# E3SM-Project/tinman_sandbox

Measured on NVIDIA B200. Metric: compute_and_apply_rhs_elem_lev_updates_per_s, higher is better.
Workload: dtype f64

## Files before the change

tinman_sandbox_b200/csrc/caar_capi.cu:

```cuda
#include <cstdarg>
#include <cstddef>
#include <cstdio>
#include <cstdlib>
#include <cstring>
#include <initializer_list>
#include <new>

#include "caar_device.cuh"

#ifndef CAAR_HOST_DEFAULT_ZERO_COPY
#define CAAR_HOST_DEFAULT_ZERO_COPY 0
#endif

namespace {

thread_local char g_err[512] = "";

int fail(int code, const char* fmt, ...) {
  va_list ap;
  va_start(ap, fmt);
  vsnprintf(g_err, sizeof g_err, fmt, ap);
  va_end(ap);
  return code;
}
// ... 37 lines not shown
  unsigned long long* bits;
  double* out3;
  double* out3_host;
  cudaEvent_t ev0, ev1;
  long long launches;
  caar::TmaMaps* tma;
  cudaStream_t s_in, s_in2, s_out;
  cudaEvent_t* chunk_ev;
  int n_chunk_ev;
  cudaEvent_t ev_fence;
  int rsplit;
  double* hybi_dev;
  double* extra[5];
  double* stage;
  unsigned* lapflat_sched;
  caar::TmaMaps* tma_host;
  double* tma_host_key[CAAR_NUM_FIELDS];
};

static_assert(sizeof(caar_arrays) == CAAR_NUM_FIELDS * sizeof(double*), "caar_arrays must be 16 pointers");
static_assert(sizeof(caar_dims) == 20 && offsetof(caar_dims, nlev) == 4 && offsetof(caar_dims, ntl) == 16, "caar_dims: 5 ints");
static_assert(offsetof(caar_arrays, elem_state_dp3d) == 48 && offsetof(caar_arrays, elem_derived_vn0) == 120,
              "caar_arrays: the order of struct Arrays");
static_assert(sizeof(caar_constants) == 48 && offsetof(caar_constants, kappa) == 40, "caar_constants: 6 doubles");
static_assert(sizeof(caar_control) == 32 && offsetof(caar_control, qn0) == 20 && offsetof(caar_control, dt2) == 24,
              "caar_control: 6 ints + 1 double");
static_assert(sizeof(caar_checksum) == 184 && offsetof(caar_checksum, sumsq) == 56 && offsetof(caar_checksum, bits) == 112 &&
                  offsetof(caar_checksum, energy) == 168,
              "caar_checksum: 7 + 7 doubles, 7 64-bit integers, 2 doubles");

// ... 46 lines not shown
  a.metdet = ptr[4]; a.rmetdet = ptr[5]; a.dp3d = ptr[6]; a.v = ptr[7];
  a.T = ptr[8]; a.phis = ptr[9]; a.Qdp = ptr[10]; a.eta_dot_dpdn = ptr[11];
  a.omega_p = ptr[12]; a.phi = ptr[13]; a.pecnd = ptr[14]; a.vn0 = ptr[15];
  a.nelem = h->dims.nelem; a.nlev = h->dims.nlev; a.qsize_d = h->dims.qsize_d; a.ntl = h->dims.ntl;
  if (ctl) {
    a.nets = ctl->nets; a.nete = ctl->nete; a.n0 = ctl->n0; a.np1 = ctl->np1; a.nm1 = ctl->nm1;
    a.qn0 = ctl->qn0; a.dt2 = ctl->dt2;
  }
  a.rrearth = h->c.rrearth; a.eta_ave_w = h->c.eta_ave_w; a.Rwv = h->c.Rwater_vapor; a.Rgas = h->c.Rgas;
  a.kappa = h->c.kappa; a.hyai0 = h->hyai0; a.ps0 = h->ps0;
  for (int i = 0; i < 16; ++i) a.dvv[i] = h->dvv[i];
  a.tma = h->tma;
  a.rsplit = h->rsplit;
  a.hybi = h->hybi_dev;
  a.lapflat_sched = h->lapflat_sched;
  return a;
}

}

extern "C" {

const char* caar_last_error(void) { return g_err; }
const char* caar_version(void) { return "caar_b200 0.1 (sm_100a)"; }

size_t caar_field_count(const caar_dims* dims, int f) {
  if (!dims || f < 0 || f >= CAAR_NUM_FIELDS) return 0;
  return field_count(*dims, f);
}

// ... 32 lines not shown
  if (e == cudaSuccess) e = cudaEventCreateWithFlags(&h->ev_fence, cudaEventDisableTiming);
  if (e == cudaSuccess) e = cudaStreamCreateWithFlags(&h->s_in, cudaStreamNonBlocking);
  if (e == cudaSuccess) e = cudaStreamCreateWithFlags(&h->s_in2, cudaStreamNonBlocking);
  if (e == cudaSuccess) e = cudaStreamCreateWithFlags(&h->s_out, cudaStreamNonBlocking);
  for (int f = 0; f < CAAR_NUM_FIELDS && e == cudaSuccess; ++f) {
    const size_t bytes = field_count(*dims, f) * sizeof(double);
    e = cudaMalloc(&h->dev[f], bytes);
    if (e == cudaSuccess) e = cudaMemsetAsync(h->dev[f], 0, bytes, h->own_stream);
  }
  if (e == cudaSuccess) e = cudaMalloc(&h->partial, (size_t)dims->nelem * 16 * sizeof(double));
  if (e == cudaSuccess) e = cudaMalloc(&h->bits, (size_t)dims->nelem * 7 * sizeof(unsigned long long));
  if (e == cudaSuccess) e = cudaMalloc(&h->out3, 23 * sizeof(double));
  if (e == cudaSuccess) e = cudaMallocHost(&h->out3_host, 23 * sizeof(double));
  if (e == cudaSuccess) e = cudaMalloc(&h->lapflat_sched, 2 * sizeof(unsigned));
  if (e == cudaSuccess) e = cudaMemsetAsync(h->lapflat_sched, 0, 2 * sizeof(unsigned), h->own_stream);
  if (e == cudaSuccess) e = cudaStreamSynchronize(h->own_stream);
  if (e != cudaSuccess) {
    const int code = fail(e == cudaErrorMemoryAllocation ? CAAR_ERR_NOMEM : CAAR_ERR_CUDA, "caar_create: %s",
                          cudaGetErrorString(e));
    char keep[sizeof g_err];
    std::memcpy(keep, g_err, sizeof keep);
    caar_destroy(h);
    std::memcpy(g_err, keep, sizeof keep);
    cudaGetLastError();
    return code;
  }
  h->stream = h->own_stream;
  h->rsplit = 1;
  if (caar::fused_supports(dims->nlev)) {
    h->tma = new (std::nothrow) caar::TmaMaps();
// ... 10 lines not shown
int caar_destroy(caar_handle h) {
  if (!h) return CAAR_OK;
  DeviceGuard guard(h->device);
  if (h->own_stream) cudaStreamSynchronize(h->own_stream);
  for (int f = 0; f < CAAR_NUM_FIELDS; ++f)
    if (h->dev[f]) cudaFree(h->dev[f]);
  if (h->partial) cudaFree(h->partial);
  if (h->bits) cudaFree(h->bits);
  if (h->out3) cudaFree(h->out3);
  if (h->stage) cudaFree(h->stage);
  for (int x = 0; x < CAAR_NUM_EXTRA; ++x)
    if (h->extra[x]) cudaFree(h->extra[x]);
  if (h->hybi_dev) cudaFree(h->hybi_dev);
  if (h->out3_host) cudaFreeHost(h->out3_host);
  if (h->lapflat_sched) cudaFree(h->lapflat_sched);
  if (h->ev0) cudaEventDestroy(h->ev0);
  if (h->ev1) cudaEventDestroy(h->ev1);
  if (h->ev_fence) cudaEventDestroy(h->ev_fence);
  for (int i = 0; i < h->n_chunk_ev; ++i) cudaEventDestroy(h->chunk_ev[i]);
  delete[] h->chunk_ev;
  if (h->s_in) cudaStreamSynchronize(h->s_in), cudaStreamDestroy(h->s_in);
  if (h->s_in2) cudaStreamSynchronize(h->s_in2), cudaStreamDestroy(h->s_in2);
  if (h->s_out) cudaStreamSynchronize(h->s_out), cudaStreamDestroy(h->s_out);
  if (h->own_stream) cudaStreamDestroy(h->own_stream);
  delete h->tma;
  delete h->tma_host;
  delete h;
  return CAAR_OK;
}

// ... 723 lines not shown
```

tinman_sandbox_b200/csrc/caar_device.cuh:

```cuda
#pragma once
#include <cstddef>
#include <cstdint>
#include <cuda.h>
#include <cuda_runtime.h>

#include "caar_b200.h"

namespace caar {

constexpr int NP = 4;
constexpr int PTS = 16;

struct KernelArgs {
  const double* D;
  const double* Dinv;
  const double* fcor;
  const double* spheremp;
  const double* metdet;
  const double* rmetdet;
  double* dp3d;
  double* v;
  double* T;
  const double* phis;
  const double* Qdp;
// ... 1 lines not shown
  double* omega_p;
  double* phi;
  const double* pecnd;
  double* vn0;
  int nelem, nlev, qsize_d, ntl;
  int nets, nete, n0, np1, nm1, qn0;
  double dt2;
  double rrearth, eta_ave_w, Rwv, Rgas, kappa;
  double hyai0, ps0;
  double dvv[16];
  const void* tma;
  int rsplit;
  const double* hybi;
  int pf_dist;
  unsigned* lapflat_sched;
};

struct alignas(64) TmaMaps {
  CUtensorMap dp3d, T, v, vn0, pecnd, omega_p, phi, Qdp;
};
int build_tma_maps(TmaMaps* out, const KernelArgs& a, char* err, size_t errlen);

cudaError_t launch_strict(const KernelArgs& a, cudaStream_t s);
cudaError_t launch_fused(const KernelArgs& a, cudaStream_t s);
bool fused_supports(int nlev);
bool fused_supports_eulerian(int nlev);
int fused_instance_levels(int nlev);
int fused_instance_cluster(int nlev);
cudaError_t launch_fused_more(const KernelArgs& a, cudaStream_t s);
size_t strict_smem_bytes(int nlev);
// ... 20 lines not shown
```

tinman_sandbox_b200/csrc/caar_fused.cu:

```cuda
#include "caar_fused_kernel.cuh"

namespace caar {
int build_tma_maps(TmaMaps* out, const KernelArgs& a, char* err, size_t errlen) {
  typedef CUresult (*encode_t)(CUtensorMap*, CUtensorMapDataType, cuuint32_t, void*, const cuuint64_t*,
                               const cuuint64_t*, const cuuint32_t*, const cuuint32_t*, CUtensorMapInterleave,
                               CUtensorMapSwizzle, CUtensorMapL2promotion, CUtensorMapFloatOOBfill);
  void* fn = nullptr;
  cudaDriverEntryPointQueryResult qres;
  cudaError_t ce = cudaGetDriverEntryPoint("cuTensorMapEncodeTiled", &fn, cudaEnableDefault, &qres);
  if (ce != cudaSuccess || !fn || qres != cudaDriverEntryPointSuccess) {
    snprintf(err, errlen, "cuTensorMapEncodeTiled entry point unavailable (%s)", cudaGetErrorString(ce));
    return 1;
  }
  const encode_t encode = reinterpret_cast<encode_t>(fn);
  const cuuint64_t E = (cuuint64_t)a.nelem, L = (cuuint64_t)a.nlev, ntl = (cuuint64_t)a.ntl;
  const int inst = instance_for(a.nlev);
  const cuuint32_t LB = (cuuint32_t)(inst / (cluster_for(inst) > 0 ? cluster_for(inst) : 1));
  struct Spec { CUtensorMap* m; const void* base; cuuint64_t slices; cuuint64_t rows; cuuint32_t box; const char* name; };
  const Spec specs[8] = {
      {&out->Qdp, a.Qdp, E * (cuuint64_t)a.qsize_d * 2, L, LB, "Qdp"},
      {&out->dp3d, a.dp3d, E * ntl, L, LB, "dp3d"},
      {&out->T, a.T, E * ntl, L, LB, "T"},
      {&out->v, a.v, E * ntl, 2 * L, 2 * LB, "v"},
      {&out->vn0, a.vn0, E, 2 * L, 2 * LB, "vn0"},
// ... 19 lines not shown
      return 1;
    }
  }
  return 0;
}

bool fused_supports_eulerian(int nlev) { return instance_for(nlev) > 0; }

bool fused_supports(int nlev) { return instance_for(nlev) > 0; }

int fused_instance_levels(int nlev) { return instance_for(nlev); }
int fused_instance_cluster(int nlev) { return instance_for(nlev) ? cluster_for(instance_for(nlev)) : 0; }

cudaError_t launch_fused(const KernelArgs& a0, cudaStream_t s) {
  KernelArgs a = a0;
  static const int pf_env = [] {
    const char* v = getenv("CAAR_PF_DIST");
    return v ? atoi(v) : -1;
  }();
  a.pf_dist = a0.pf_dist < 0 ? 0 : (pf_env >= 0 ? pf_env : (a.nlev == 72 ? sm_count() / 2 : 32));
  switch (instance_for(a.nlev)) {
    case 72: return launch_nlev<72>(a, s);
    case 128: return launch_nlev<128>(a, s);
    case 0: return cudaErrorInvalidValue;
  }
  return launch_fused_more(a, s);
}

}
```

tinman_sandbox_b200/csrc/caar_fused_kernel.cuh:

```cuda
#pragma once
#include <cstdio>
#include <cstdlib>

#include "caar_device.cuh"

namespace caar {
namespace {

constexpr unsigned FULL = 0xffffffffu;

__device__ __forceinline__ uint32_t smem_u32(const void* p) { return (uint32_t)__cvta_generic_to_shared(p); }
__device__ __forceinline__ void mbar_init(uint64_t* bar, unsigned count) {
  asm volatile("mbarrier.init.shared::cta.b64 [%0], %1;" ::"r"(smem_u32(bar)), "r"(count) : "memory");
}
__device__ __forceinline__ void fence_proxy_async() { asm volatile("fence.proxy.async.shared::cta;" ::: "memory"); }
__device__ __forceinline__ void mbar_expect_tx(uint64_t* bar, unsigned bytes) {
  asm volatile("mbarrier.arrive.expect_tx.shared::cta.b64 _, [%0], %1;" ::"r"(smem_u32(bar)), "r"(bytes) : "memory");
}
__device__ __forceinline__ void tma_load(void* dst, const CUtensorMap* map, int row, int slice, uint64_t* bar) {
  asm volatile(
      "cp.async.bulk.tensor.3d.shared::cluster.global.tile.mbarrier::complete_tx::bytes [%0], [%1, {%2, %3, %4}], [%5];" ::"r"(
          smem_u32(dst)),
      "l"(map), "r"(0), "r"(row), "r"(slice), "r"(smem_u32(bar))
      : "memory");
}
__device__ __forceinline__ void mbar_wait(uint64_t* bar, unsigned parity) {
  const uint32_t addr = smem_u32(bar);
  uint32_t done;
  do {
    asm volatile(
        "{ .reg .pred p; mbarrier.try_wait.parity.shared::cta.b64 p, [%1], %2; selp.u32 %0, 1, 0, p; }"
        : "=r"(done)
        : "r"(addr), "r"(parity)
        : "memory");
  } while (!done);
}
__device__ __forceinline__ void tma_store(const CUtensorMap* map, int row, int slice, const void* src) {
  asm volatile("cp.async.bulk.tensor.3d.global.shared::cta.tile.bulk_group [%0, {%1, %2, %3}], [%4];" ::"l"(map), "r"(0),
               "r"(row), "r"(slice), "r"(smem_u32(src))
               : "memory");
}
__device__ __forceinline__ void prefetch_l2(const void* p, unsigned bytes) {
  asm volatile("cp.async.bulk.prefetch.L2.global [%0], %1;" ::"l"(p), "r"(bytes) : "memory");
}
__device__ __forceinline__ void bulk_commit() { asm volatile("cp.async.bulk.commit_group;" ::: "memory"); }
__device__ __forceinline__ void bulk_wait_read_all() { asm volatile("cp.async.bulk.wait_group.read 0;" ::: "memory"); }

__device__ __forceinline__ uint32_t cluster_ctarank() {
  uint32_t r;
  asm volatile("mov.u32 %0, %%cluster_ctarank;" : "=r"(r));
// ... 3 lines not shown
__device__ __forceinline__ void cluster_arrive_relaxed() { asm volatile("barrier.cluster.arrive.relaxed.aligned;" ::: "memory"); }
__device__ __forceinline__ void cluster_wait() { asm volatile("barrier.cluster.wait.acquire.aligned;" ::: "memory"); }
__device__ __forceinline__ void fence_mbar_init_cluster() { asm volatile("fence.mbarrier_init.release.cluster;" ::: "memory"); }
__device__ __forceinline__ void st_row_async_remote(const double* local, const uint64_t* bar, uint32_t rank,
                                                    const double (&x)[4]) {
  uint32_t dst, rbar;
  asm volatile("mapa.shared::cluster.u32 %0, %1, %2;" : "=r"(dst) : "r"(smem_u32(local)), "r"(rank));
  asm volatile("mapa.shared::cluster.u32 %0, %1, %2;" : "=r"(rbar) : "r"(smem_u32(bar)), "r"(rank));
  asm volatile("st.async.weak.shared::cluster.mbarrier::complete_tx::bytes.v2.f64 [%0], {%1, %2}, [%3];" ::"r"(dst),
               "d"(x[0]), "d"(x[1]), "r"(rbar)
               : "memory");
  asm volatile("st.async.weak.shared::cluster.mbarrier::complete_tx::bytes.v2.f64 [%0], {%1, %2}, [%3];" ::"r"(dst + 16),
               "d"(x[2]), "d"(x[3]), "r"(rbar)
               : "memory");
}

__device__ __forceinline__ double fast_rcp(double x) {
  double r;
  asm("rcp.approx.ftz.f64 %0, %1;" : "=d"(r) : "d"(x));
  r = fma(fma(-x, r, 1.0), r, r);
  r = fma(fma(-x, r, 1.0), r, r);
  return r;
}

struct Row {
  double x[4];
};
__device__ __forceinline__ Row ld_row(const double* p) {
  const double2 a = *reinterpret_cast<const double2*>(p);
  const double2 b = *reinterpret_cast<const double2*>(p + 2);
// ... 195 lines not shown
  }
  a0 += a1;
  t0 += t1;
  a0 += __shfl_xor_sync(FULL, a0, 16);
  t0 += __shfl_xor_sync(FULL, t0, 16);
#pragma unroll
  for (int j = 0; j < 4; ++j) {
    pre[j] = __shfl_sync(FULL, a0, r * 4 + j);
    all[j] = __shfl_sync(FULL, t0, r * 4 + j);
  }
}

#ifndef CAAR_PARK
#define CAAR_PARK 1
#endif
#ifndef CAAR_EUL_HOIST
#define CAAR_EUL_HOIST 56
#endif
#ifndef CAAR_CL72
#define CAAR_CL72 3
#endif
#ifndef CAAR_CL128
#define CAAR_CL128 2
#endif
#ifndef CAAR_REGS_SMALL
#define CAAR_REGS_SMALL 96
#endif

__host__ __device__ constexpr int cluster_for(int nlev) {
  return nlev == 72 ? CAAR_CL72 : nlev == 128 ? CAAR_CL128
// ... 14 lines not shown

__host__ __device__ constexpr bool park_for(int L, int CL, bool eul) { return CAAR_PARK && L == 72 && CL == 1 && !eul; }

template <int L, int NWT, bool EUL, bool PARK = false>
struct Smem {
  static constexpr int LF = L * PTS;
  double vn0[2 * LF];
  double vm1[2 * LF];
  double pec[LF];
  double omp[LF];
  double dpm[LF];
  double Tm1[LF];
  double Tn0[LF];
  double Qd[LF];
  double vn[EUL ? 2 * LF : 2];
  double tot[3][NWT][16];
  double dinv[4 * 20];
  double dmat[4 * 20];
  double met[16], rmet[16], fcor[16], mp[16], phis[16];
  uint64_t bar[3];
  uint64_t xbar[3];
};

template <int L, int CL, bool EUL>
__global__ void __launch_bounds__(4 * L / CL) __maxnreg__(regs_for(4 * L / CL, EUL))
caar_fused_kernel(const __grid_constant__ KernelArgs A, const __grid_constant__ TmaMaps M) {
  constexpr int LC = L / CL;
  constexpr int NW = LC / 8;
  constexpr int NWT = L / 8;
  constexpr int LF = LC * PTS;
  constexpr int GS = 20;
  constexpr unsigned FB = LF * sizeof(double);
  static_assert(L % (8 * CL) == 0, "a warp holds 8 levels");
  extern __shared__ __align__(1024) unsigned char smem_raw[];
  constexpr bool PARK = park_for(L, CL, EUL);
  Smem<LC, NWT, EUL, PARK>& S = *reinterpret_cast<Smem<LC, NWT, EUL, PARK>*>(smem_raw + ((1024u - (smem_u32(smem_raw) & 1023u)) & 1023u));

  const int t = threadIdx.x;
  const int lane = t & 31, w = t >> 5;
  const int r = t & 3;
  const uint32_t rank = (CL > 1) ? cluster_ctarank() : 0u;
  const int gw = (int)rank * NW + w;
  const int lev0 = (int)rank * LC;
  const int ie = A.nets + (int)(blockIdx.x / CL);
  const size_t e = (size_t)ie;
  const int nl = A.nlev;
  const size_t lf = (size_t)nl * PTS;
  const int off = lev0 * PTS + t * 4;
  const bool live = lev0 + (t >> 2) < nl;
  const uint32_t sw1 = (uint32_t)(t >> 2) * 128u + ((uint32_t)((2 * r) ^ ((t >> 2) & 7)) << 4);
  const uint32_t sw2 = (uint32_t)(t >> 1) * 128u + ((uint32_t)((4 * (r & 1)) ^ ((t >> 1) & 7)) << 4);
  const int sl_n0 = ie * A.ntl + A.n0, sl_nm1 = ie * A.ntl + A.nm1, sl_np1 = ie * A.ntl + A.np1;

  if (t == 0) {
    mbar_init(&S.bar[0], 1);
    mbar_init(&S.bar[1], 1);
    mbar_init(&S.bar[2], 1);
    if (CL > 1) {
      constexpr unsigned XB = NW * 16 * sizeof(double);
      mbar_init(&S.xbar[0], 1);
      mbar_init(&S.xbar[1], 1);
      mbar_init(&S.xbar[2], 1);
      fence_mbar_init_cluster();
      if (rank > 0) {
        mbar_expect_tx(&S.xbar[0], rank * XB);
        mbar_expect_tx(&S.xbar[2], rank * XB);
      }
      if (rank + 1 < CL) mbar_expect_tx(&S.xbar[1], (CL - 1 - rank) * (EUL ? 2 * XB : XB));
    }
    fence_proxy_async();
  }
  if (CL > 1) cluster_arrive_relaxed();
  if (t == 0) {
    mbar_expect_tx(&S.bar[2], ((A.qn0 != -1 ? 2 : 1) + (EUL ? 2 : 0)) * FB);
    tma_load(S.Tn0, &M.T, lev0, sl_n0, &S.bar[2]);
    if (EUL) tma_load(S.vn, &M.v, lev0 * 2, sl_n0, &S.bar[2]);
    if (A.qn0 != -1) tma_load(S.Qd, &M.Qdp, lev0, (ie * A.qsize_d + 0) * 2 + A.qn0, &S.bar[2]);
    mbar_expect_tx(&S.bar[0], 4 * FB);
    tma_load(S.vn0, &M.vn0, lev0 * 2, ie, &S.bar[0]);
    tma_load(S.dpm, &M.dp3d, lev0, sl_nm1, &S.bar[0]);
    tma_load(S.pec, &M.pecnd, lev0, ie, &S.bar[0]);
    mbar_expect_tx(&S.bar[1], 4 * FB);
    tma_load(S.omp, &M.omega_p, lev0, ie, &S.bar[1]);
    tma_load(S.Tm1, &M.T, lev0, sl_nm1, &S.bar[1]);
    tma_load(S.vm1, &M.v, lev0 * 2, sl_nm1, &S.bar[1]);
    const int pe = ie + A.pf_dist;
    if (A.pf_dist > 0 && pe < A.nete && lev0 < nl) {
      const size_t pn0 = ((size_t)pe * A.ntl + A.n0) * lf + (size_t)lev0 * PTS;
      const unsigned PB = (nl - lev0 < LC) ? (unsigned)(nl - lev0) * PTS * sizeof(double) : FB;
      prefetch_l2(A.dp3d + pn0, PB);
      prefetch_l2(A.v + pn0 * 2, 2 * PB);
      prefetch_l2(A.T + pn0, PB);
      if (A.qn0 != -1) prefetch_l2(A.Qdp + (((size_t)pe * A.qsize_d + 0) * 2 + A.qn0) * lf + (size_t)lev0 * PTS, PB);
      if (rank == 0) {
        prefetch_l2(A.Dinv + (size_t)pe * 64, 512);
        prefetch_l2(A.D + (size_t)pe * 64, 512);
        prefetch_l2(A.metdet + (size_t)pe * 16, 128);
        prefetch_l2(A.rmetdet + (size_t)pe * 16, 128);
        prefetch_l2(A.fcor + (size_t)pe * 16, 128);
        prefetch_l2(A.spheremp + (size_t)pe * 16, 128);
        prefetch_l2(A.phis + (size_t)pe * 16, 128);
      }
    }
  }

  const size_t on0 = (e * A.ntl + A.n0) * lf + off;
  Row dp, v1, v2;
  if (live) {
    dp = ld_row(A.dp3d + on0);
    ld_row2(A.v + on0 * 2, v1, v2);
  } else {
#pragma unroll
    for (int j = 0; j < 4; ++j) dp.x[j] = 1.0, v1.x[j] = 0.0, v2.x[j] = 0.0;
  }
  if (EUL && r == 0 && live)
    asm volatile("prefetch.global.L2 [%0];" ::"l"(A.eta_dot_dpdn + e * (lf + PTS) + off));

  for (int g = t; g < 96; g += 4 * LC) {
    if (g < 64) {
      S.dinv[(g >> 4) * GS + (g & 15)] = A.Dinv[e * 64 + g] * A.rrearth;
      S.dmat[(g >> 4) * GS + (g & 15)] = A.D[e * 64 + g];
    } else if (g < 80) {
      const int q = g - 64;
      S.met[q] = A.metdet[e * 16 + q];
      S.rmet[q] = A.rmetdet[e * 16 + q];
      S.fcor[q] = A.fcor[e * 16 + q];
    } else {
      const int q = g - 80;
      S.mp[q] = A.spheremp[e * 16 + q];
      S.phis[q] = A.phis[e * 16 + q];
    }
  }

#if CAAR_DERIV_MMA
  const DerivMma cx = deriv_mma_setup(A.dvv, lane);
#else
  double cx[4];
#pragma unroll
  for (int x = 0; x < 4; ++x) {
    double c = A.dvv[(0 ^ x) * 4 + 0];
    if (r == 1) c = A.dvv[(1 ^ x) * 4 + 1];
    if (r == 2) c = A.dvv[(2 ^ x) * 4 + 2];
    if (r == 3) c = A.dvv[(3 ^ x) * 4 + 3];
    cx[x] = c;
  }
#endif

  Row rp;
  {
    Row p;
#pragma unroll
    for (int j = 0; j < 4; ++j) p.x[j] = scan_down(dp.x[j], lane);
    if (CL > 1) cluster_wait();
    if (lane >= 28) {
      st_row(&S.tot[0][gw][r * 4], p);
      if (CL > 1)
        for (uint32_t rr = rank + 1; rr < (uint32_t)CL; ++rr) st_row_async_remote(&S.tot[0][gw][r * 4], &S.xbar[0], rr, p.x);
    }
    __syncthreads();
    if (CL > 1 && rank > 0) mbar_wait(&S.xbar[0], 0);
    constexpr bool LANE_CARRY = (CL > 1) || (NWT >= 16) || EUL;
    double carry[4] = {0, 0, 0, 0};
    if constexpr (LANE_CARRY) {
      warp_totals<NWT>(S.tot[0], 0, gw, lane, carry);
    } else {
#pragma unroll
      for (int ww = 0; ww < NWT - 1; ++ww)
        if (ww < gw) {
          const Row c = ld_row(&S.tot[0][ww][r * 4]);
#pragma unroll
          for (int j = 0; j < 4; ++j) carry[j] += c.x[j];
        }
    }
    const double ptop = A.hyai0 * A.ps0;
#pragma unroll
    for (int j = 0; j < 4; ++j) {
      p.x[j] = ptop + ((carry[j] + p.x[j]) - 0.5 * dp.x[j]);
      rp.x[j] = fast_rcp(p.x[j]);
    }

    Row fv;
    {
      Row vc0, vc1;
#pragma unroll
// ... 14 lines not shown
    constexpr bool FUSE_W = (CL > 1);
    Row w1, w2;
    if constexpr (FUSE_W) {
      const Row a = deriv_i(p, cx), b = deriv_j(p, A.dvv);
#pragma unroll
      for (int j = 0; j < 4; ++j) {
        const double2 d01 = lds2(S.dinv + r * GS + j * 4), d23 = lds2(S.dinv + r * GS + j * 4 + 2);
        gp0.x[j] = fma(d01.x, a.x[j], d23.x * b.x[j]);
        gp1.x[j] = fma(d01.y, a.x[j], d23.y * b.x[j]);
        w1.x[j] = fma(d01.x, v1.x[j], d01.y * v2.x[j]);
        w2.x[j] = fma(d23.x, v1.x[j], d23.y * v2.x[j]);
      }
    } else {
      gradient(p, S.dinv + r * GS, cx, A.dvv, gp0, gp1);
    }
    mbar_wait(&S.bar[2], 0);
    Row Tv = ld_tile(S.Tn0, sw1);
    if (A.qn0 != -1) {
      const Row Qd = ld_tile(S.Qd, sw1);
      const double c = A.Rwv / A.Rgas - 1.0;
#pragma unroll
      for (int j = 0; j < 4; ++j) Tv.x[j] *= fma(c, Qd.x[j] * fast_rcp(dp.x[j]), 1.0);
    }
#pragma unroll
    for (int j = 0; j < 4; ++j) {
      const double vg = fma(v1.x[j], gp0.x[j], v2.x[j] * gp1.x[j]);
      const double gl = -A.Rgas * (Tv.x[j] * rp.x[j]);
      gp0.x[j] = fma(gl, gp0.x[j], v2.x[j] * fv.x[j]);
      gp1.x[j] = fma(gl, gp1.x[j], -v1.x[j] * fv.x[j]);
      p.x[j] = vg;
    }
// ... 11 lines not shown
      }
    }
    Row ttp;
    {
      const Row T = ld_tile(S.Tn0, sw1);
      const Row a = deriv_i(T, cx), b = deriv_j(T, A.dvv);
#pragma unroll
      for (int j = 0; j < 4; ++j) ttp.x[j] = -fma(a.x[j], w1.x[j], b.x[j] * w2.x[j]);
    }
    if (PARK) {
      st_tile(S.Tn0, sw1, vt1);
      st_tile(S.Qd, sw1, vt2);
    }
    if (EUL) st_tile(S.Qd, sw1, vt2);

    mbar_wait(&S.bar[0], 0);

    Row divdp;
    {
      {
        Row a0, a1;
        ld_tile2(S.vn0, sw2, a0, a1);
#pragma unroll
        for (int j = 0; j < 4; ++j) {
          a0.x[j] = fma(A.eta_ave_w, v1.x[j] * dp.x[j], a0.x[j]);
          a1.x[j] = fma(A.eta_ave_w, v2.x[j] * dp.x[j], a1.x[j]);
        }
        st_tile2(S.vn0, sw2, a0, a1);
      }
      const Row met = ld_row(S.met + r * 4);
#pragma unroll
// ... 31 lines not shown
    Row a, ph;
    {
      Row tq;
      const Row phis = ld_row(S.phis + r * 4);
#pragma unroll
      for (int j = 0; j < 4; ++j) {
        const double q = A.Rgas * Tv.x[j] * (dp.x[j] * rp.x[j]);
        const double sq = scan_up(q, lane);
        const double sd = scan_down(divdp.x[j], lane);
        ph.x[j] = phis.x[j] + (sq - 0.5 * q);
        a.x[j] = rp.x[j] * (vgp.x[j] - (sd - 0.5 * divdp.x[j]));
        tq.x[j] = sq;
        divdp.x[j] = sd;
      }
      if (lane < 4) {
        st_row(&S.tot[1][gw][r * 4], tq);
        if (CL > 1)
          for (uint32_t rr = 0; rr < rank; ++rr) st_row_async_remote(&S.tot[1][gw][r * 4], &S.xbar[1], rr, tq.x);
      }
      if (lane >= 28) {
        st_row(&S.tot[2][gw][r * 4], divdp);
        if (CL > 1) {
          for (uint32_t rr = rank + 1; rr < (uint32_t)CL; ++rr)
            st_row_async_remote(&S.tot[2][gw][r * 4], &S.xbar[2], rr, divdp.x);
          if (EUL)
            for (uint32_t rr = 0; rr < rank; ++rr) st_row_async_remote(&S.tot[2][gw][r * 4], &S.xbar[1], rr, divdp.x);
        }
      }
    }
    Row tta, ttb;
#pragma unroll
    for (int j = 0; j < 4; ++j) {
      const double kt = A.kappa * Tv.x[j];
      tta.x[j] = fma(kt, a.x[j], ttp.x[j]);
      ttb.x[j] = kt * rp.x[j];
    }
    __syncthreads();
    if (CL > 1) {
      if (rank + 1 < CL) mbar_wait(&S.xbar[1], 0);
      if (rank > 0) mbar_wait(&S.xbar[2], 0);
    }
    if (t == 0) {
      tma_store(&M.vn0, lev0 * 2, ie, S.vn0);
      if (!EUL) tma_store(&M.dp3d, lev0, sl_np1, S.dpm);
      bulk_commit();
    }
    double cq[4] = {0, 0, 0, 0}, cd[4] = {0, 0, 0, 0};
    double S4[4] = {0, 0, 0, 0};
    if constexpr (LANE_CARRY) {
      warp_totals<NWT>(S.tot[1], gw + 1, NWT, lane, cq);
      if constexpr (EUL && CAAR_WT_BOTH && NWT <= 12) warp_totals_both<NWT>(S.tot[2], gw, lane, cd, S4);
      else warp_totals<NWT>(S.tot[2], 0, gw, lane, cd);
    } else {
#pragma unroll
      for (int ww = 0; ww < NWT; ++ww) {
        if (ww > gw) {
          const Row c = ld_row(&S.tot[1][ww][r * 4]);
#pragma unroll
          for (int j = 0; j < 4; ++j) cq[j] += c.x[j];
        }
        if (ww < gw) {
          const Row c = ld_row(&S.tot[2][ww][r * 4]);
#pragma unroll
          for (int j = 0; j < 4; ++j) cd[j] += c.x[j];
        }
      }
    }

    mbar_wait(&S.bar[1], 0);
    const Row mp = ld_row(S.mp + r * 4);
    Row eta_old, dpk_early;
    constexpr bool HOIST = EUL && (CAAR_EUL_HOIST > 0) && (LC >= CAAR_EUL_HOIST);
    if (EUL) {
      if (HOIST && live) {
        dpk_early = ld_row(A.dp3d + on0);
        if (lev0 + (t >> 2) > 0) eta_old = ld_row(A.eta_dot_dpdn + e * (lf + PTS) + off);
      }
      {
        Row om = ld_tile(S.omp, sw1);
#pragma unroll
        for (int j = 0; j < 4; ++j) {
          om.x[j] = fma(A.eta_ave_w, fma(-rp.x[j], cd[j], a.x[j]), om.x[j]);
          tta.x[j] = fma(-ttb.x[j], cd[j], tta.x[j]);
        }
        st_tile(S.omp, sw1, om);
      }
      kep = ld_tile(S.pec, sw1);
#pragma unroll
      for (int j = 0; j < 4; ++j) {
        ph.x[j] += cq[j];
        kep.x[j] += ph.x[j];
      }
      st_tile(S.pec, sw1, ph);
      if constexpr (LANE_CARRY) {
        if constexpr (!(CAAR_WT_BOTH && NWT <= 12)) warp_totals<NWT>(S.tot[2], 0, NWT, lane, S4);
      } else {
#pragma unroll
        for (int ww = 0; ww < NWT; ++ww) {
          const Row c = ld_row(&S.tot[2][ww][r * 4]);
#pragma unroll
          for (int j = 0; j < 4; ++j) S4[j] += c.x[j];
        }
      }
      const int kg = lev0 + (t >> 2);
      const double hb_lo = A.hybi[kg < nl ? kg : nl], hb_hi = A.hybi[kg < nl ? kg + 1 : nl];
      Row ehi, elo;
#pragma unroll
      for (int j = 0; j < 4; ++j) {
        const double P = cd[j] + divdp.x[j];
        ehi.x[j] = (kg >= nl - 1) ? 0.0 : fma(hb_hi, S4[j], -P);
        elo.x[j] = (kg == 0) ? 0.0 : fma(hb_lo, S4[j], -(P - dsave.x[j]));
      }
      {
        Row o = ld_tile(S.dpm, sw1);
// ... 93 lines not shown
#pragma unroll
      for (int j = 0; j < 4; ++j) {
        a0.x[j] = mp.x[j] * fma(A.dt2, vt1.x[j] - g0.x[j], a0.x[j]);
        a1.x[j] = mp.x[j] * fma(A.dt2, vt2.x[j] - g1.x[j], a1.x[j]);
      }
      st_tile2(S.vm1, sw2, a0, a1);
    }
  }
  fence_proxy_async();
  if (CL > 1 && EUL && A.np1 == A.n0) {
    cluster_arrive();
    cluster_wait();
  } else {
    __syncthreads();
  }
  if (t == 0) {
    if (EUL) tma_store(&M.dp3d, lev0, sl_np1, S.dpm);
    tma_store(&M.omega_p, lev0, ie, S.omp);
    tma_store(&M.T, lev0, sl_np1, S.Tm1);
    tma_store(&M.phi, lev0, ie, S.pec);
    tma_store(&M.v, lev0 * 2, sl_np1, S.vm1);
    bulk_commit();
    bulk_wait_read_all();
  }
}

template <int L, int CL, bool EUL>
cudaError_t launch_L(const KernelArgs& a, cudaStream_t s) {
  static_assert((4 * L / CL) * regs_for(4 * L / CL, EUL) <= 65536, "one CTA must fit the 64K-register file of an SM");
  const int n = a.nete - a.nets;
  if (n <= 0) return cudaSuccess;
  constexpr int SMEM = (int)sizeof(Smem<L / CL, L / 8, EUL, park_for(L, CL, EUL)>) + 1024;
  static bool configured[64] = {};
  int dev = 0;
  cudaError_t e = cudaGetDevice(&dev);
  if (e != cudaSuccess) return e;
  if (dev < 0 || dev >= 64 || !configured[dev]) {
    e = cudaFuncSetAttribute(caar_fused_kernel<L, CL, EUL>, cudaFuncAttributeMaxDynamicSharedMemorySize, SMEM);
    if (e != cudaSuccess) return e;
    e = cudaFuncSetAttribute(caar_fused_kernel<L, CL, EUL>, cudaFuncAttributePreferredSharedMemoryCarveout,
                             (int)cudaSharedmemCarveoutMaxShared);
    if (e != cudaSuccess) return e;
    if (dev >= 0 && dev < 64) configured[dev] = true;
  }
  if (!a.tma) return cudaErrorInvalidValue;
  static const bool debug_occ = getenv("CAAR_DEBUG_OCC") != nullptr;
  if (debug_occ) {
    int nb = -1;
    cudaOccupancyMaxActiveBlocksPerMultiprocessor(&nb, caar_fused_kernel<L, CL, EUL>, 4 * L / CL, SMEM);
    fprintf(stderr, "[caar] caar_fused_kernel<%d,%d,%d>: %d threads, %d B dynamic smem -> %d CTAs/SM\n", L, CL, (int)EUL,
            4 * L / CL, SMEM, nb);
  }
  cudaLaunchConfig_t cfg = {};
  cfg.gridDim = dim3((unsigned)n * CL, 1, 1);
  cfg.blockDim = dim3(4 * L / CL, 1, 1);
  cfg.dynamicSmemBytes = SMEM;
  cfg.stream = s;
  cudaLaunchAttribute attr[2];
  attr[0].id = cudaLaunchAttributeClusterDimension;
  attr[0].val.clusterDim.x = CL;
  attr[0].val.clusterDim.y = 1;
  attr[0].val.clusterDim.z = 1;
  static const int policy_env = [] { const char* v = getenv("CAAR_CLUSTER_POLICY"); return v ? atoi(v) : 0; }();
  const bool balance = policy_env ? (policy_env == 2) : (CL >= 3);
  attr[1].id = cudaLaunchAttributeClusterSchedulingPolicyPreference;
  attr[1].val.clusterSchedulingPolicyPreference =
      balance ? cudaClusterSchedulingPolicyLoadBalancing : cudaClusterSchedulingPolicySpread;
  cfg.attrs = attr;
  cfg.numAttrs = (CL > 1) ? 2 : 0;
  return cudaLaunchKernelEx(&cfg, caar_fused_kernel<L, CL, EUL>, a, *static_cast<const TmaMaps*>(a.tma));
}

template <int L>
cudaError_t launch_nlev(const KernelArgs& a, cudaStream_t s) {
  static_assert(cluster_for(L) > 0, "no fused instance for this level count");
  return a.rsplit == 0 ? launch_L<L, cluster_for(L), true>(a, s) : launch_L<L, cluster_for(L), false>(a, s);
}

}
}
```

Baseline: 2.570 billion.

## Make non-Eulerian fused kernel persistent with atomic element scheduling and cross-element prefetch

For the rsplit!=0 path, the fused kernel now launches only as many clusters as can be resident and loops over elements. Each cluster draws its next element from a global atomic counter, and rank 0 broadcasts that choice to the other ranks over DSMEM. TMA loads for the next element are issued while the current element's stores drain, and the cluster-exchange buffers and mbarriers are double-buffered with phase tracking. The aim is to remove per-CTA launch and prologue cost and hide load latency. In exchange it adds atomics, a counter reset at kernel end, and more shared memory and barrier phase complexity, which could lower occupancy or introduce ordering bugs.

```diff
diff --git a/tinman_sandbox_b200/csrc/caar_capi.cu b/tinman_sandbox_b200/csrc/caar_capi.cu
--- a/tinman_sandbox_b200/csrc/caar_capi.cu
+++ b/tinman_sandbox_b200/csrc/caar_capi.cu
@@ -75,6 +75,7 @@
   double* extra[5];
   double* stage;
   unsigned* lapflat_sched;
+  unsigned* fused_sched;
   caar::TmaMaps* tma_host;
   double* tma_host_key[CAAR_NUM_FIELDS];
 };
@@ -151,6 +152,7 @@
   a.rsplit = h->rsplit;
   a.hybi = h->hybi_dev;
   a.lapflat_sched = h->lapflat_sched;
+  a.fused_sched = h->fused_sched;
   return a;
 }
 
@@ -213,6 +215,8 @@
   if (e == cudaSuccess) e = cudaMallocHost(&h->out3_host, 23 * sizeof(double));
   if (e == cudaSuccess) e = cudaMalloc(&h->lapflat_sched, 2 * sizeof(unsigned));
   if (e == cudaSuccess) e = cudaMemsetAsync(h->lapflat_sched, 0, 2 * sizeof(unsigned), h->own_stream);
+  if (e == cudaSuccess) e = cudaMalloc(&h->fused_sched, 2 * sizeof(unsigned));
+  if (e == cudaSuccess) e = cudaMemsetAsync(h->fused_sched, 0, 2 * sizeof(unsigned), h->own_stream);
   if (e == cudaSuccess) e = cudaStreamSynchronize(h->own_stream);
   if (e != cudaSuccess) {
     const int code = fail(e == cudaErrorMemoryAllocation ? CAAR_ERR_NOMEM : CAAR_ERR_CUDA, "caar_create: %s",
@@ -253,6 +257,7 @@
   if (h->hybi_dev) cudaFree(h->hybi_dev);
   if (h->out3_host) cudaFreeHost(h->out3_host);
   if (h->lapflat_sched) cudaFree(h->lapflat_sched);
+  if (h->fused_sched) cudaFree(h->fused_sched);
   if (h->ev0) cudaEventDestroy(h->ev0);
   if (h->ev1) cudaEventDestroy(h->ev1);
   if (h->ev_fence) cudaEventDestroy(h->ev_fence);
diff --git a/tinman_sandbox_b200/csrc/caar_device.cuh b/tinman_sandbox_b200/csrc/caar_device.cuh
--- a/tinman_sandbox_b200/csrc/caar_device.cuh
+++ b/tinman_sandbox_b200/csrc/caar_device.cuh
@@ -39,6 +39,8 @@
   const double* hybi;
   int pf_dist;
   unsigned* lapflat_sched;
+  unsigned* fused_sched;
+  long long* timeline;
 };
 
 struct alignas(64) TmaMaps {
diff --git a/tinman_sandbox_b200/csrc/caar_fused.cu b/tinman_sandbox_b200/csrc/caar_fused.cu
--- a/tinman_sandbox_b200/csrc/caar_fused.cu
+++ b/tinman_sandbox_b200/csrc/caar_fused.cu
@@ -1,6 +1,9 @@
 #include "caar_fused_kernel.cuh"
 
 namespace caar {
+#if CAAR_FUSED_TIMELINE
+static long long* g_timeline = nullptr;
+#endif
 int build_tma_maps(TmaMaps* out, const KernelArgs& a, char* err, size_t errlen) {
   typedef CUresult (*encode_t)(CUtensorMap*, CUtensorMapDataType, cuuint32_t, void*, const cuuint64_t*,
                                const cuuint64_t*, const cuuint32_t*, const cuuint32_t*, CUtensorMapInterleave,
@@ -57,6 +60,9 @@
 
 cudaError_t launch_fused(const KernelArgs& a0, cudaStream_t s) {
   KernelArgs a = a0;
+#if CAAR_FUSED_TIMELINE
+  a.timeline = g_timeline;
+#endif
   static const int pf_env = [] {
     const char* v = getenv("CAAR_PF_DIST");
     return v ? atoi(v) : -1;
@@ -71,3 +77,7 @@
 }
 
 }
+
+#if CAAR_FUSED_TIMELINE
+extern "C" void caar_fused_timeline(long long* buf) { caar::g_timeline = buf; }
+#endif
diff --git a/tinman_sandbox_b200/csrc/caar_fused_kernel.cuh b/tinman_sandbox_b200/csrc/caar_fused_kernel.cuh
--- a/tinman_sandbox_b200/csrc/caar_fused_kernel.cuh
+++ b/tinman_sandbox_b200/csrc/caar_fused_kernel.cuh
@@ -24,16 +24,30 @@
       "l"(map), "r"(0), "r"(row), "r"(slice), "r"(smem_u32(bar))
       : "memory");
 }
-__device__ __forceinline__ void mbar_wait(uint64_t* bar, unsigned parity) {
+#ifndef CAAR_MBAR_WAIT_BOUND
+#define CAAR_MBAR_WAIT_BOUND 0
+#endif
+__device__ __forceinline__ void mbar_wait(uint64_t* bar, unsigned parity, int elem = -1) {
   const uint32_t addr = smem_u32(bar);
   uint32_t done;
+#if CAAR_MBAR_WAIT_BOUND
+  unsigned tries = 0;
+#endif
   do {
     asm volatile(
         "{ .reg .pred p; mbarrier.try_wait.parity.shared::cta.b64 p, [%1], %2; selp.u32 %0, 1, 0, p; }"
         : "=r"(done)
         : "r"(addr), "r"(parity)
         : "memory");
+#if CAAR_MBAR_WAIT_BOUND
+    if (!done && ++tries == (1u << 26)) {
+      printf("[caar] mbar_wait timeout: block %u thread %u barrier smem 0x%x parity %u element %d\n", blockIdx.x, threadIdx.x,
+             addr, parity, elem);
+      return;
+    }
+#endif
   } while (!done);
+  (void)elem;
 }
 __device__ __forceinline__ void tma_store(const CUtensorMap* map, int row, int slice, const void* src) {
   asm volatile("cp.async.bulk.tensor.3d.global.shared::cta.tile.bulk_group [%0, {%1, %2, %3}], [%4];" ::"l"(map), "r"(0),
@@ -67,6 +81,13 @@
                "d"(x[2]), "d"(x[3]), "r"(rbar)
                : "memory");
 }
+__device__ __forceinline__ void st_int_async_remote(const int* local, const uint64_t* bar, uint32_t rank, int x) {
+  uint32_t dst, rbar;
+  asm volatile("mapa.shared::cluster.u32 %0, %1, %2;" : "=r"(dst) : "r"(smem_u32(local)), "r"(rank));
+  asm volatile("mapa.shared::cluster.u32 %0, %1, %2;" : "=r"(rbar) : "r"(smem_u32(bar)), "r"(rank));
+  asm volatile("st.async.weak.shared::cluster.mbarrier::complete_tx::bytes.b32 [%0], %1, [%2];" ::"r"(dst), "r"(x), "r"(rbar)
+               : "memory");
+}
 
 __device__ __forceinline__ double fast_rcp(double x) {
   double r;
@@ -292,6 +313,15 @@
 #ifndef CAAR_PARK
 #define CAAR_PARK 1
 #endif
+#ifndef CAAR_PERSIST_STAGGER
+#define CAAR_PERSIST_STAGGER 0
+#endif
+#ifndef CAAR_PERSIST_SCHED
+#define CAAR_PERSIST_SCHED 1
+#endif
+#ifndef CAAR_FUSED_TIMELINE
+#define CAAR_FUSED_TIMELINE 0
+#endif
 #ifndef CAAR_EUL_HOIST
 #define CAAR_EUL_HOIST 56
 #endif
@@ -336,12 +366,13 @@
   double Tn0[LF];
   double Qd[LF];
   double vn[EUL ? 2 * LF : 2];
-  double tot[3][NWT][16];
+  double tot[EUL ? 1 : 2][3][NWT][16];
   double dinv[4 * 20];
   double dmat[4 * 20];
   double met[16], rmet[16], fcor[16], mp[16], phis[16];
   uint64_t bar[3];
-  uint64_t xbar[3];
+  uint64_t xbar[EUL ? 1 : 2][3];
+  int nxt[2];
 };
 
 template <int L, int CL, bool EUL>
@@ -364,49 +395,35 @@
   const uint32_t rank = (CL > 1) ? cluster_ctarank() : 0u;
   const int gw = (int)rank * NW + w;
   const int lev0 = (int)rank * LC;
-  const int ie = A.nets + (int)(blockIdx.x / CL);
-  const size_t e = (size_t)ie;
   const int nl = A.nlev;
   const size_t lf = (size_t)nl * PTS;
   const int off = lev0 * PTS + t * 4;
   const bool live = lev0 + (t >> 2) < nl;
   const uint32_t sw1 = (uint32_t)(t >> 2) * 128u + ((uint32_t)((2 * r) ^ ((t >> 2) & 7)) << 4);
   const uint32_t sw2 = (uint32_t)(t >> 1) * 128u + ((uint32_t)((4 * (r & 1)) ^ ((t >> 1) & 7)) << 4);
-  const int sl_n0 = ie * A.ntl + A.n0, sl_nm1 = ie * A.ntl + A.nm1, sl_np1 = ie * A.ntl + A.np1;
-
-  if (t == 0) {
-    mbar_init(&S.bar[0], 1);
-    mbar_init(&S.bar[1], 1);
-    mbar_init(&S.bar[2], 1);
-    if (CL > 1) {
-      constexpr unsigned XB = NW * 16 * sizeof(double);
-      mbar_init(&S.xbar[0], 1);
-      mbar_init(&S.xbar[1], 1);
-      mbar_init(&S.xbar[2], 1);
-      fence_mbar_init_cluster();
-      if (rank > 0) {
-        mbar_expect_tx(&S.xbar[0], rank * XB);
-        mbar_expect_tx(&S.xbar[2], rank * XB);
-      }
-      if (rank + 1 < CL) mbar_expect_tx(&S.xbar[1], (CL - 1 - rank) * (EUL ? 2 * XB : XB));
-    }
-    fence_proxy_async();
-  }
-  if (CL > 1) cluster_arrive_relaxed();
-  if (t == 0) {
+  constexpr unsigned XB = NW * 16 * sizeof(double);
+  const auto arm_x0 = [&](int p) { mbar_expect_tx(&S.xbar[p][0], rank * XB + (EUL ? 0u : 4u)); };
+  const auto arm_x1 = [&](int p) { mbar_expect_tx(&S.xbar[p][1], (CL - 1 - rank) * (EUL ? 2 * XB : XB)); };
+  const auto arm_x2 = [&](int p) { mbar_expect_tx(&S.xbar[p][2], rank * XB); };
+  const auto load_b2 = [&](int el) {
     mbar_expect_tx(&S.bar[2], ((A.qn0 != -1 ? 2 : 1) + (EUL ? 2 : 0)) * FB);
-    tma_load(S.Tn0, &M.T, lev0, sl_n0, &S.bar[2]);
-    if (EUL) tma_load(S.vn, &M.v, lev0 * 2, sl_n0, &S.bar[2]);
-    if (A.qn0 != -1) tma_load(S.Qd, &M.Qdp, lev0, (ie * A.qsize_d + 0) * 2 + A.qn0, &S.bar[2]);
+    tma_load(S.Tn0, &M.T, lev0, el * A.ntl + A.n0, &S.bar[2]);
+    if (EUL) tma_load(S.vn, &M.v, lev0 * 2, el * A.ntl + A.n0, &S.bar[2]);
+    if (A.qn0 != -1) tma_load(S.Qd, &M.Qdp, lev0, (el * A.qsize_d + 0) * 2 + A.qn0, &S.bar[2]);
+  };
+  const auto load_b0a = [&](int el) {
     mbar_expect_tx(&S.bar[0], 4 * FB);
-    tma_load(S.vn0, &M.vn0, lev0 * 2, ie, &S.bar[0]);
-    tma_load(S.dpm, &M.dp3d, lev0, sl_nm1, &S.bar[0]);
-    tma_load(S.pec, &M.pecnd, lev0, ie, &S.bar[0]);
+    tma_load(S.vn0, &M.vn0, lev0 * 2, el, &S.bar[0]);
+    tma_load(S.dpm, &M.dp3d, lev0, el * A.ntl + A.nm1, &S.bar[0]);
+  };
+  const auto load_b0b = [&](int el) { tma_load(S.pec, &M.pecnd, lev0, el, &S.bar[0]); };
+  const auto load_b1 = [&](int el) {
     mbar_expect_tx(&S.bar[1], 4 * FB);
-    tma_load(S.omp, &M.omega_p, lev0, ie, &S.bar[1]);
-    tma_load(S.Tm1, &M.T, lev0, sl_nm1, &S.bar[1]);
-    tma_load(S.vm1, &M.v, lev0 * 2, sl_nm1, &S.bar[1]);
-    const int pe = ie + A.pf_dist;
+    tma_load(S.omp, &M.omega_p, lev0, el, &S.bar[1]);
+    tma_load(S.Tm1, &M.T, lev0, el * A.ntl + A.nm1, &S.bar[1]);
+    tma_load(S.vm1, &M.v, lev0 * 2, el * A.ntl + A.nm1, &S.bar[1]);
+  };
+  const auto prefetch_elem = [&](int pe) {
     if (A.pf_dist > 0 && pe < A.nete && lev0 < nl) {
       const size_t pn0 = ((size_t)pe * A.ntl + A.n0) * lf + (size_t)lev0 * PTS;
       const unsigned PB = (nl - lev0 < LC) ? (unsigned)(nl - lev0) * PTS * sizeof(double) : FB;
@@ -424,7 +441,77 @@
         prefetch_l2(A.phis + (size_t)pe * 16, 128);
       }
     }
-  }
+  };
+
+  constexpr int NXP = EUL ? 1 : 2;
+  if (t == 0) {
+    mbar_init(&S.bar[0], 1);
+    mbar_init(&S.bar[1], 1);
+    mbar_init(&S.bar[2], 1);
+    if (CL > 1) {
+#pragma unroll
+      for (int p = 0; p < NXP; ++p) {
+        mbar_init(&S.xbar[p][0], 1);
+        mbar_init(&S.xbar[p][1], 1);
+        mbar_init(&S.xbar[p][2], 1);
+      }
+      fence_mbar_init_cluster();
+#pragma unroll
+      for (int p = 0; p < NXP; ++p) {
+        if (rank > 0) arm_x0(p), arm_x2(p);
+        if (rank + 1 < CL) arm_x1(p);
+      }
+    }
+    fence_proxy_async();
+  }
+  if (CL > 1) cluster_arrive_relaxed();
+  int ie = A.nets + (int)(blockIdx.x / CL);
+#if CAAR_PERSIST_STAGGER
+  if (!EUL) __nanosleep((unsigned)((blockIdx.x / CL) % 5) * CAAR_PERSIST_STAGGER);
+#endif
+  if (t == 0) {
+    load_b2(ie);
+    load_b0a(ie);
+    load_b0b(ie);
+    load_b1(ie);
+    if (EUL) prefetch_elem(ie + A.pf_dist);
+  }
+
+#if CAAR_DERIV_MMA
+  const DerivMma cx = deriv_mma_setup(A.dvv, lane);
+#else
+  double cx[4];
+#pragma unroll
+  for (int x = 0; x < 4; ++x) {
+    double c = A.dvv[(0 ^ x) * 4 + 0];
+    if (r == 1) c = A.dvv[(1 ^ x) * 4 + 1];
+    if (r == 2) c = A.dvv[(2 ^ x) * 4 + 2];
+    if (r == 3) c = A.dvv[(3 ^ x) * 4 + 3];
+    cx[x] = c;
+  }
+#endif
+
+#if CAAR_FUSED_TIMELINE
+  long long tl_entry = clock64(), tl_math = 0, tl_bar = 0;
+#endif
+#if CAAR_PERSIST_SCHED == 1
+  int ahead = ie + (int)(gridDim.x / CL);
+#endif
+  for (unsigned it = 0;; ++it) {
+  const unsigned bph = EUL ? 0u : (it & 1u);
+  const int xp = EUL ? 0 : (int)(it & 1u);
+  const unsigned xph = EUL ? 0u : ((it >> 1) & 1u);
+  const size_t e = (size_t)ie;
+  const int sl_np1 = ie * A.ntl + A.np1;
+#if CAAR_PERSIST_SCHED == 0
+  int drawn = 0;
+  if (!EUL && rank == 0 && t == 0) drawn = A.nets + (int)(gridDim.x / CL) + (int)atomicAdd(A.fused_sched, 1u);
+#elif CAAR_PERSIST_SCHED == 1
+  const int drawn = ahead;
+  if (!EUL && rank == 0 && t == 0 && drawn < A.nete) ahead = A.nets + 2 * (int)(gridDim.x / CL) + (int)atomicAdd(A.fused_sched, 1u);
+#else
+  const int drawn = ie + (int)(gridDim.x / CL);
+#endif
 
   const size_t on0 = (e * A.ntl + A.n0) * lf + off;
   Row dp, v1, v2;
@@ -454,42 +541,39 @@
     }
   }
 
-#if CAAR_DERIV_MMA
-  const DerivMma cx = deriv_mma_setup(A.dvv, lane);
-#else
-  double cx[4];
-#pragma unroll
-  for (int x = 0; x < 4; ++x) {
-    double c = A.dvv[(0 ^ x) * 4 + 0];
-    if (r == 1) c = A.dvv[(1 ^ x) * 4 + 1];
-    if (r == 2) c = A.dvv[(2 ^ x) * 4 + 2];
-    if (r == 3) c = A.dvv[(3 ^ x) * 4 + 3];
-    cx[x] = c;
-  }
-#endif
-
   Row rp;
   {
     Row p;
 #pragma unroll
     for (int j = 0; j < 4; ++j) p.x[j] = scan_down(dp.x[j], lane);
-    if (CL > 1) cluster_wait();
+#if CAAR_FUSED_TIMELINE
+    if (t == 0) tl_math = clock64();
+#endif
+    if (CL > 1 && it == 0) cluster_wait();
     if (lane >= 28) {
-      st_row(&S.tot[0][gw][r * 4], p);
+      st_row(&S.tot[xp][0][gw][r * 4], p);
       if (CL > 1)
-        for (uint32_t rr = rank + 1; rr < (uint32_t)CL; ++rr) st_row_async_remote(&S.tot[0][gw][r * 4], &S.xbar[0], rr, p.x);
+        for (uint32_t rr = rank + 1; rr < (uint32_t)CL; ++rr) st_row_async_remote(&S.tot[xp][0][gw][r * 4], &S.xbar[xp][0], rr, p.x);
+    }
+    if (!EUL && rank == 0 && t == 0) {
+      S.nxt[xp] = drawn;
+      for (uint32_t rr = 1; rr < (uint32_t)CL; ++rr) st_int_async_remote(&S.nxt[xp], &S.xbar[xp][0], rr, drawn);
     }
     __syncthreads();
-    if (CL > 1 && rank > 0) mbar_wait(&S.xbar[0], 0);
+    if (CL > 1 && rank > 0) {
+      mbar_wait(&S.xbar[xp][0], xph, ie);
+      if (!EUL && t == 0) arm_x0(xp);
+    }
+    if (!EUL && t == 0) prefetch_elem(S.nxt[xp]);
     constexpr bool LANE_CARRY = (CL > 1) || (NWT >= 16) || EUL;
     double carry[4] = {0, 0, 0, 0};
     if constexpr (LANE_CARRY) {
-      warp_totals<NWT>(S.tot[0], 0, gw, lane, carry);
+      warp_totals<NWT>(S.tot[xp][0], 0, gw, lane, carry);
     } else {
 #pragma unroll
       for (int ww = 0; ww < NWT - 1; ++ww)
         if (ww < gw) {
-          const Row c = ld_row(&S.tot[0][ww][r * 4]);
+          const Row c = ld_row(&S.tot[xp][0][ww][r * 4]);
 #pragma unroll
           for (int j = 0; j < 4; ++j) carry[j] += c.x[j];
         }
@@ -534,7 +618,7 @@
     } else {
       gradient(p, S.dinv + r * GS, cx, A.dvv, gp0, gp1);
     }
-    mbar_wait(&S.bar[2], 0);
+    mbar_wait(&S.bar[2], bph, ie);
     Row Tv = ld_tile(S.Tn0, sw1);
     if (A.qn0 != -1) {
       const Row Qd = ld_tile(S.Qd, sw1);
@@ -576,7 +660,7 @@
     }
     if (EUL) st_tile(S.Qd, sw1, vt2);
 
-    mbar_wait(&S.bar[0], 0);
+    mbar_wait(&S.bar[0], bph, ie);
 
     Row divdp;
     {
@@ -638,17 +722,17 @@
         divdp.x[j] = sd;
       }
       if (lane < 4) {
-        st_row(&S.tot[1][gw][r * 4], tq);
+        st_row(&S.tot[xp][1][gw][r * 4], tq);
         if (CL > 1)
-          for (uint32_t rr = 0; rr < rank; ++rr) st_row_async_remote(&S.tot[1][gw][r * 4], &S.xbar[1], rr, tq.x);
+          for (uint32_t rr = 0; rr < rank; ++rr) st_row_async_remote(&S.tot[xp][1][gw][r * 4], &S.xbar[xp][1], rr, tq.x);
       }
       if (lane >= 28) {
-        st_row(&S.tot[2][gw][r * 4], divdp);
+        st_row(&S.tot[xp][2][gw][r * 4], divdp);
         if (CL > 1) {
           for (uint32_t rr = rank + 1; rr < (uint32_t)CL; ++rr)
-            st_row_async_remote(&S.tot[2][gw][r * 4], &S.xbar[2], rr, divdp.x);
+            st_row_async_remote(&S.tot[xp][2][gw][r * 4], &S.xbar[xp][2], rr, divdp.x);
           if (EUL)
-            for (uint32_t rr = 0; rr < rank; ++rr) st_row_async_remote(&S.tot[2][gw][r * 4], &S.xbar[1], rr, divdp.x);
+            for (uint32_t rr = 0; rr < rank; ++rr) st_row_async_remote(&S.tot[xp][2][gw][r * 4], &S.xbar[xp][1], rr, divdp.x);
         }
       }
     }
@@ -661,37 +745,48 @@
     }
     __syncthreads();
     if (CL > 1) {
-      if (rank + 1 < CL) mbar_wait(&S.xbar[1], 0);
-      if (rank > 0) mbar_wait(&S.xbar[2], 0);
+      if (rank + 1 < CL) {
+        mbar_wait(&S.xbar[xp][1], xph, ie);
+        if (!EUL && t == 0) arm_x1(xp);
+      }
+      if (rank > 0) {
+        mbar_wait(&S.xbar[xp][2], xph, ie);
+        if (!EUL && t == 0) arm_x2(xp);
+      }
     }
     if (t == 0) {
       tma_store(&M.vn0, lev0 * 2, ie, S.vn0);
       if (!EUL) tma_store(&M.dp3d, lev0, sl_np1, S.dpm);
       bulk_commit();
+      if (!EUL && !PARK && S.nxt[xp] < A.nete) {
+        fence_proxy_async();
+        load_b2(S.nxt[xp]);
+      }
+
     }
     double cq[4] = {0, 0, 0, 0}, cd[4] = {0, 0, 0, 0};
     double S4[4] = {0, 0, 0, 0};
     if constexpr (LANE_CARRY) {
-      warp_totals<NWT>(S.tot[1], gw + 1, NWT, lane, cq);
-      if constexpr (EUL && CAAR_WT_BOTH && NWT <= 12) warp_totals_both<NWT>(S.tot[2], gw, lane, cd, S4);
-      else warp_totals<NWT>(S.tot[2], 0, gw, lane, cd);
+      warp_totals<NWT>(S.tot[xp][1], gw + 1, NWT, lane, cq);
+      if constexpr (EUL && CAAR_WT_BOTH && NWT <= 12) warp_totals_both<NWT>(S.tot[xp][2], gw, lane, cd, S4);
+      else warp_totals<NWT>(S.tot[xp][2], 0, gw, lane, cd);
     } else {
 #pragma unroll
       for (int ww = 0; ww < NWT; ++ww) {
         if (ww > gw) {
-          const Row c = ld_row(&S.tot[1][ww][r * 4]);
+          const Row c = ld_row(&S.tot[xp][1][ww][r * 4]);
 #pragma unroll
           for (int j = 0; j < 4; ++j) cq[j] += c.x[j];
         }
         if (ww < gw) {
-          const Row c = ld_row(&S.tot[2][ww][r * 4]);
+          const Row c = ld_row(&S.tot[xp][2][ww][r * 4]);
 #pragma unroll
           for (int j = 0; j < 4; ++j) cd[j] += c.x[j];
         }
       }
     }
 
-    mbar_wait(&S.bar[1], 0);
+    mbar_wait(&S.bar[1], bph, ie);
     const Row mp = ld_row(S.mp + r * 4);
     Row eta_old, dpk_early;
     constexpr bool HOIST = EUL && (CAAR_EUL_HOIST > 0) && (LC >= CAAR_EUL_HOIST);
@@ -717,11 +812,11 @@
       }
       st_tile(S.pec, sw1, ph);
       if constexpr (LANE_CARRY) {
-        if constexpr (!(CAAR_WT_BOTH && NWT <= 12)) warp_totals<NWT>(S.tot[2], 0, NWT, lane, S4);
+        if constexpr (!(CAAR_WT_BOTH && NWT <= 12)) warp_totals<NWT>(S.tot[xp][2], 0, NWT, lane, S4);
       } else {
 #pragma unroll
         for (int ww = 0; ww < NWT; ++ww) {
-          const Row c = ld_row(&S.tot[2][ww][r * 4]);
+          const Row c = ld_row(&S.tot[xp][2][ww][r * 4]);
 #pragma unroll
           for (int j = 0; j < 4; ++j) S4[j] += c.x[j];
         }
@@ -845,6 +940,9 @@
   } else {
     __syncthreads();
   }
+#if CAAR_FUSED_TIMELINE
+  if (t == 0) tl_bar = clock64();
+#endif
   if (t == 0) {
     if (EUL) tma_store(&M.dp3d, lev0, sl_np1, S.dpm);
     tma_store(&M.omega_p, lev0, ie, S.omp);
@@ -853,6 +951,34 @@
     tma_store(&M.v, lev0 * 2, sl_np1, S.vm1);
     bulk_commit();
     bulk_wait_read_all();
+    if (!EUL && S.nxt[xp] < A.nete) {
+      if (PARK) load_b2(S.nxt[xp]);
+      load_b0a(S.nxt[xp]);
+      load_b0b(S.nxt[xp]);
+      load_b1(S.nxt[xp]);
+    }
+  }
+#if CAAR_FUSED_TIMELINE
+  if (t == 0 && A.timeline) {
+    const long long tl_exit = clock64();
+    unsigned smid;
+    asm volatile("mov.u32 %0, %%smid;" : "=r"(smid));
+    long long* rec = A.timeline + ((size_t)(ie - A.nets) * CL + rank) * 5;
+    rec[0] = smid, rec[1] = tl_entry, rec[2] = tl_math, rec[3] = tl_bar, rec[4] = tl_exit;
+    tl_entry = tl_exit;
+  }
+#endif
+  if (EUL) break;
+  ie = S.nxt[xp];
+  if (ie >= A.nete) break;
+  }
+  if (!EUL && CAAR_PERSIST_SCHED < 2 && rank == 0 && t == 0) {
+    __threadfence();
+    const unsigned done = atomicAdd(A.fused_sched + 1, 1u);
+    if (done == gridDim.x / CL - 1) {
+      A.fused_sched[0] = 0;
+      A.fused_sched[1] = 0;
+    }
   }
 }
 
@@ -863,6 +989,7 @@
   if (n <= 0) return cudaSuccess;
   constexpr int SMEM = (int)sizeof(Smem<L / CL, L / 8, EUL, park_for(L, CL, EUL)>) + 1024;
   static bool configured[64] = {};
+  static int resident_clusters[64] = {};
   int dev = 0;
   cudaError_t e = cudaGetDevice(&dev);
   if (e != cudaSuccess) return e;
@@ -882,6 +1009,7 @@
     fprintf(stderr, "[caar] caar_fused_kernel<%d,%d,%d>: %d threads, %d B dynamic smem -> %d CTAs/SM\n", L, CL, (int)EUL,
             4 * L / CL, SMEM, nb);
   }
+  if (!EUL && !a.fused_sched) return cudaErrorInvalidValue;
   cudaLaunchConfig_t cfg = {};
   cfg.gridDim = dim3((unsigned)n * CL, 1, 1);
   cfg.blockDim = dim3(4 * L / CL, 1, 1);
@@ -899,6 +1027,22 @@
       balance ? cudaClusterSchedulingPolicyLoadBalancing : cudaClusterSchedulingPolicySpread;
   cfg.attrs = attr;
   cfg.numAttrs = (CL > 1) ? 2 : 0;
+  if (!EUL) {
+    int& nc = resident_clusters[(dev >= 0 && dev < 64) ? dev : 0];
+    if (nc <= 0 || dev < 0 || dev >= 64) {
+      if (CL > 1) {
+        e = cudaOccupancyMaxActiveClusters(&nc, caar_fused_kernel<L, CL, EUL>, &cfg);
+      } else {
+        int per_sm = 0;
+        e = cudaOccupancyMaxActiveBlocksPerMultiprocessor(&per_sm, caar_fused_kernel<L, CL, EUL>, 4 * L / CL, SMEM);
+        nc = per_sm * sm_count();
+      }
+      if (e != cudaSuccess) return e;
+      if (nc <= 0) return cudaErrorInvalidConfiguration;
+    }
+    cfg.gridDim = dim3((unsigned)(n < nc ? n : nc) * CL, 1, 1);
+    if (debug_occ) fprintf(stderr, "[caar] caar_fused_kernel<%d,%d,%d>: %d resident clusters\n", L, CL, (int)EUL, nc);
+  }
   return cudaLaunchKernelEx(&cfg, caar_fused_kernel<L, CL, EUL>, a, *static_cast<const TmaMaps*>(a.tma));
 }
 
```

Result: slower. 2.433 billion, median of 6 (-5.3%).
